# dusk-network/dusk-blindbidproof

Measured on AMD Instinct MI355X. Metric: blind-bid proofs/sec, higher is better.
Workload: dtype u32

## Files before the change

### __graft_entry__.py

```python
import os
import shutil
import subprocess
import sys

ROOT = os.path.dirname(os.path.abspath(__file__))
PKG = os.path.join(ROOT, "dusk_blindbidproof_amd")
CSRC = os.path.join(PKG, "csrc")
LIB = os.path.join(PKG, "libbbp_hip.so")
ORACLE_SO = os.path.join(ROOT, "oracle", "_build", "libbbp_oracle.so")
HOSTCHECK_SO = os.path.join(ROOT, "tests", "_build", "libhostcheck.so")
DEVCHECK_SO = {"chain": os.path.join(ROOT, "tests", "_build", "libbbp_devcheck.so"),
               "nochain": os.path.join(ROOT, "tests", "_build", "libbbp_devcheck_nochain.so")}
DEVCHECK_DEFS = {"chain": [], "nochain": ["-DBBP_FE_NO_CHAIN"]}


def _newer(target, sources):
    if not os.path.exists(target):
        return True
    t = os.path.getmtime(target)
    return any(os.path.getmtime(s) > t for s in sources)


def _run(cmd):
    print("+", " ".join(cmd), flush=True)
    subprocess.check_call(cmd)


def _csrc_files(exts):
    return sorted(os.path.join(CSRC, f) for f in os.listdir(CSRC) if f.endswith(exts))


def build_hip(force=False):
    srcs = _csrc_files((".hip", ".cpp"))
    deps = srcs + _csrc_files((".h", ".inc")) + [os.path.join(ROOT, "include", "bbp.h")]
    if not force and not _newer(LIB, deps):
        return LIB
    hipcc = shutil.which("hipcc") or "/opt/rocm/bin/hipcc"
    objdir = os.path.join(PKG, "build")
    os.makedirs(objdir, exist_ok=True)
    objs = []
    procs = []
    for s in srcs:
        o = os.path.join(objdir, os.path.basename(s) + ".o")
        objs.append(o)
        if force or _newer(o, [s] + _csrc_files((".h", ".inc")) + [os.path.join(ROOT, "include", "bbp.h")]):
            cmd = [hipcc, "--offload-arch=gfx950", "-O3", "-std=c++17", "-fPIC", "-c", s, "-o", o]
            print("+", " ".join(cmd), flush=True)
            procs.append((cmd, subprocess.Popen(cmd)))
    for cmd, p in procs:
        if p.wait() != 0:
            raise subprocess.CalledProcessError(p.returncode, cmd)
    _run([hipcc, "--offload-arch=gfx950", "-shared", "-fPIC", "-o", LIB] + objs)
    return LIB


def stale_artefacts():
    stale = []
    deps = _csrc_files((".hip", ".cpp", ".h", ".inc")) + [os.path.join(ROOT, "include", "bbp.h")]
    if _newer(LIB, deps):
        stale.append(os.path.relpath(LIB, ROOT))
    odir = os.path.join(ROOT, "oracle", "c")
    if _newer(ORACLE_SO, [os.path.join(odir, f) for f in os.listdir(odir)]):
        stale.append(os.path.relpath(ORACLE_SO, ROOT))
    return stale


def build_oracle(force=False):
    src = os.path.join(ROOT, "oracle", "c", "bbp_oracle.c")
    if not os.path.exists(src):
        return None
    deps = [os.path.join(ROOT, "oracle", "c", f) for f in os.listdir(os.path.join(ROOT, "oracle", "c"))]
    if not force and not _newer(ORACLE_SO, deps):
        return ORACLE_SO
    os.makedirs(os.path.dirname(ORACLE_SO), exist_ok=True)
    _run(["gcc", "-O2", "-std=gnu11", "-shared", "-fPIC", "-pthread", "-o", ORACLE_SO, src])
    return ORACLE_SO


def build_hostcheck(force=False):
    src = os.path.join(ROOT, "tests", "host_check.cpp")
    deps = [src] + _csrc_files((".h", ".inc"))
    if not force and not _newer(HOSTCHECK_SO, deps):
        return HOSTCHECK_SO
    os.makedirs(os.path.dirname(HOSTCHECK_SO), exist_ok=True)
    _run(["g++", "-O2", "-std=c++17", "-shared", "-fPIC", "-o", HOSTCHECK_SO, src])
    return HOSTCHECK_SO


ROUNDCHECK_SO = os.path.join(ROOT, "tests", "_build", "libroundcheck.so")


def build_roundcheck(force=False):
    src = os.path.join(ROOT, "tests", "round_bids_check.cpp")
    if force or _newer(ROUNDCHECK_SO, [src] + _csrc_files((".h", ".inc"))):
        os.makedirs(os.path.dirname(ROUNDCHECK_SO), exist_ok=True)
        _run(["g++", "-O2", "-std=c++17", "-shared", "-fPIC", "-o", ROUNDCHECK_SO, src])
    return ROUNDCHECK_SO


def _devcheck_cmd(variant):
    hipcc = shutil.which("hipcc") or "/opt/rocm/bin/hipcc"
    src = os.path.join(ROOT, "tests", "device_check.hip")
    return [hipcc, "--offload-arch=gfx950", "-O3", "-std=c++17", "-fPIC", "-shared"] + DEVCHECK_DEFS[variant] + [src, "-o", DEVCHECK_SO[variant]]


def _devcheck_stale(variant):
    return _newer(DEVCHECK_SO[variant], [os.path.join(ROOT, "tests", "device_check.hip")] + _csrc_files((".h", ".inc")))


def build_devcheck(variant="chain", force=False):
    if force or _devcheck_stale(variant):
        os.makedirs(os.path.dirname(DEVCHECK_SO[variant]), exist_ok=True)
        _run(_devcheck_cmd(variant))
    return DEVCHECK_SO[variant]


def build_devcheck_all(force=False):
    procs = []
    for v in DEVCHECK_SO:
        if force or _devcheck_stale(v):
            os.makedirs(os.path.dirname(DEVCHECK_SO[v]), exist_ok=True)
            cmd = _devcheck_cmd(v)
            print("+", " ".join(cmd), flush=True)
            procs.append((cmd, subprocess.Popen(cmd)))
    for cmd, p in procs:
        if p.wait() != 0:
            raise subprocess.CalledProcessError(p.returncode, cmd)
    return dict(DEVCHECK_SO)


SERVER_BIN = os.path.join(PKG, "server", "bbp-uds-server")
LOADGEN_BIN = os.path.join(PKG, "server", "bbp-uds-loadgen")
STUB_SO = os.path.join(ROOT, "tests", "_build", "libbbp_stub.so")


def build_server(force=False):
    sdir = os.path.join(PKG, "server")
    deps = [os.path.join(sdir, f) for f in os.listdir(sdir) if f.endswith((".cpp", ".h"))] + [os.path.join(ROOT, "include", "bbp.h")]
    for out, src in ((SERVER_BIN, "uds_server.cpp"), (LOADGEN_BIN, "uds_loadgen.cpp")):
        if not os.path.exists(os.path.join(sdir, src)):
            continue
        if force or _newer(out, deps):
            _run(["g++", "-O2", "-std=c++17", "-pthread", "-o", out, os.path.join(sdir, src), "-ldl"])
    return SERVER_BIN


def build_stub_engine(force=False):
    srcs = [os.path.join(ROOT, "tests", "stub_engine.cpp"), os.path.join(CSRC, "submit.cpp")]
    if force or _newer(STUB_SO, srcs + [os.path.join(CSRC, "submit.h"), os.path.join(ROOT, "include", "bbp.h")]):
        os.makedirs(os.path.dirname(STUB_SO), exist_ok=True)
        _run(["g++", "-O2", "-std=c++17", "-shared", "-fPIC", "-pthread", "-o", STUB_SO] + srcs)
    return STUB_SO


SAN_FLAGS = {None: ["-O2"], "asan": ["-O1", "-g", "-fsanitize=address,undefined", "-fno-sanitize-recover=all"], "tsan": ["-O1", "-g", "-fsanitize=thread"]}
SERVER_SAN_BIN = {k: os.path.join(ROOT, "tests", "_build", "bbp-uds-server-" + k) for k in ("asan", "tsan")}
STUB_REFUSING_SO = {k: os.path.join(ROOT, "tests", "_build", "libbbp_stub_refusing%s.so" % ("_" + k if k else "")) for k in (None, "asan", "tsan")}


def build_server_san(kind, force=False):
    sdir = os.path.join(PKG, "server")
    deps = [os.path.join(sdir, f) for f in os.listdir(sdir) if f.endswith((".cpp", ".h"))] + [os.path.join(ROOT, "include", "bbp.h")]
    out = SERVER_SAN_BIN[kind]
    if force or _newer(out, deps):
        os.makedirs(os.path.dirname(out), exist_ok=True)
        _run(["g++"] + SAN_FLAGS[kind] + ["-std=c++17", "-pthread", "-o", out, os.path.join(sdir, "uds_server.cpp"), "-ldl"])
    return out


def build_stub_engine_refusing(kind=None, force=False):
    srcs = [os.path.join(ROOT, "tests", "stub_engine_refusing.cpp"), os.path.join(CSRC, "submit.cpp")]
# ... 34 lines not shown
    src = os.path.join(ROOT, "tests", "batch_layout_san.cpp")
    if force or _newer(BATCH_LAYOUT_SAN_BIN, [src, os.path.join(ROOT, "tests", "host_check.cpp")] + _csrc_files((".h", ".inc"))):
        os.makedirs(os.path.dirname(BATCH_LAYOUT_SAN_BIN), exist_ok=True)
        _run(["g++", "-O1", "-g", "-std=c++17", "-fsanitize=address,undefined", "-fno-sanitize-recover=all", "-o", BATCH_LAYOUT_SAN_BIN, src])
    return BATCH_LAYOUT_SAN_BIN


HEDGE_SAN_BIN = os.path.join(ROOT, "tests", "_build", "hedge_san")


def build_hedge_san(force=False):
    src = os.path.join(ROOT, "tests", "hedge_san.cpp")
    if force or _newer(HEDGE_SAN_BIN, [src] + _csrc_files((".h", ".inc"))):
        os.makedirs(os.path.dirname(HEDGE_SAN_BIN), exist_ok=True)
        _run(["g++", "-O1", "-g", "-std=c++17", "-fsanitize=address,undefined", "-fno-sanitize-recover=all", "-o", HEDGE_SAN_BIN, src])
    return HEDGE_SAN_BIN


STUB_ENTROPY_SO = os.path.join(ROOT, "tests", "_build", "libbbp_stub_entropy.so")


def build_stub_engine_entropy(force=False):
    srcs = [os.path.join(ROOT, "tests", "stub_engine_entropy.cpp"), os.path.join(CSRC, "submit.cpp")]
    if force or _newer(STUB_ENTROPY_SO, srcs + [os.path.join(ROOT, "tests", "stub_engine.cpp"), os.path.join(CSRC, "submit.h"), os.path.join(ROOT, "include", "bbp.h")]):
        os.makedirs(os.path.dirname(STUB_ENTROPY_SO), exist_ok=True)
        _run(["g++", "-O2", "-std=c++17", "-shared", "-fPIC", "-pthread", "-o", STUB_ENTROPY_SO] + srcs)
    return STUB_ENTROPY_SO


COMBINER_TSAN_BIN = os.path.join(ROOT, "tests", "_build", "combiner_tsan")


def build_combiner_tsan(force=False):
    srcs = [os.path.join(ROOT, "tests", "combiner_tsan.cpp"), os.path.join(CSRC, "submit.cpp")]
    if force or _newer(COMBINER_TSAN_BIN, srcs + [os.path.join(CSRC, "submit.h")]):
        os.makedirs(os.path.dirname(COMBINER_TSAN_BIN), exist_ok=True)
        _run(["g++", "-O1", "-g", "-std=c++17", "-fsanitize=thread", "-pthread", "-o", COMBINER_TSAN_BIN] + srcs)
    return COMBINER_TSAN_BIN


COMBINER_RULES_BIN = os.path.join(ROOT, "tests", "_build", "combiner_rules")


def build_combiner_rules(force=False):
    srcs = [os.path.join(ROOT, "tests", "combiner_rules.cpp"), os.path.join(CSRC, "submit.cpp")]
    if force or _newer(COMBINER_RULES_BIN, srcs + [os.path.join(CSRC, "submit.h")]):
        os.makedirs(os.path.dirname(COMBINER_RULES_BIN), exist_ok=True)
        _run(["g++", "-O1", "-std=c++17", "-pthread", "-o", COMBINER_RULES_BIN] + srcs)
    return COMBINER_RULES_BIN


COMBINER_MIXED_BIN = {False: os.path.join(ROOT, "tests", "_build", "combiner_mixed"), True: os.path.join(ROOT, "tests", "_build", "combiner_mixed_tsan")}


def build_combiner_mixed(tsan=False, force=False):
    out = COMBINER_MIXED_BIN[bool(tsan)]
    srcs = [os.path.join(ROOT, "tests", "combiner_mixed.cpp"), os.path.join(CSRC, "submit.cpp")]
    if force or _newer(out, srcs + [os.path.join(CSRC, "submit.h")]):
        os.makedirs(os.path.dirname(out), exist_ok=True)
        flags = ["-O1", "-g", "-fsanitize=thread"] if tsan else ["-O1"]
        _run(["g++"] + flags + ["-std=c++17", "-pthread", "-o", out] + srcs)
    return out


COMBINER_ROUNDS_BIN = {False: os.path.join(ROOT, "tests", "_build", "combiner_rounds"), True: os.path.join(ROOT, "tests", "_build", "combiner_rounds_tsan")}


def build_combiner_rounds(tsan=False, force=False):
    out = COMBINER_ROUNDS_BIN[bool(tsan)]
    srcs = [os.path.join(ROOT, "tests", "combiner_rounds.cpp"), os.path.join(CSRC, "submit.cpp")]
    if force or _newer(out, srcs + [os.path.join(CSRC, "submit.h")]):
        os.makedirs(os.path.dirname(out), exist_ok=True)
        flags = ["-O1", "-g", "-fsanitize=thread"] if tsan else ["-O1"]
        _run(["g++"] + flags + ["-std=c++17", "-pthread", "-o", out] + srcs)
    return out


def build():
    build_hip()
    build_server()
    build_stub_engine()
    build_oracle()
    build_hostcheck()
    build_roundcheck()
    build_devcheck_all()
    sys.path.insert(0, ROOT)
    import dusk_blindbidproof_amd


def smoke():
    sys.path.insert(0, ROOT)
    import dusk_blindbidproof_amd as bbp
    from tests import smoke_case

    smoke_case.run(bbp)


if __name__ == "__main__":
    build()
```

### dusk_blindbidproof_amd/csrc/msm.hip

```cpp
#include "context.h"

namespace bbp {

#ifndef BBP_FOLD_PRIO
#define BBP_FOLD_PRIO 2
#endif
#ifndef BBP_MSM_WAVES
#define BBP_MSM_WAVES 2
#endif
#ifndef BBP_MSM_WAVES_MAX
#define BBP_MSM_WAVES_MAX 2
#endif

#ifdef BBP_MSM_PROF
__device__ unsigned long long g_msm_prof[8];
#define MSM_PROF_BEGIN() unsigned long long prof_t = wall_clock64()
#define MSM_PROF_MARK(i)                                                    \
    if (tid == 0) {                                                         \
        unsigned long long now_ = wall_clock64();                           \
        atomicAdd(&g_msm_prof[i], now_ - prof_t);                           \
        prof_t = now_;                                                      \
    }
#else
#define MSM_PROF_BEGIN()
// ... 94 lines not shown
    __shared__ u32 part[SORT_T];
    const int tid = threadIdx.x;
    if (ticket && blockIdx.x == 0 && tid == 0) *ticket = 0;
    if (n_active && blockIdx.x >= *n_active) return;
    const size_t work = blockIdx.x, msm = work / split;
    const u32 i0 = (u32)(work % split) * n_sub;
    const u32 n = i0 < n_total ? min(n_sub, n_total - i0) : 0u;
    __builtin_amdgcn_s_setprio(3);
    const u32* sbase;
    const u32* base_idx = nullptr;
    u32 base0 = 0;
    if (MODE != 1) {
        const size_t src = msm_map ? (size_t)msm_map[msm] : msm;
        sbase = scal_a + (src * (size_t)n_total + i0) * 8;
        base_idx = aux + (size_t)(msm % n_idx_sets) * n_total + i0;
    } else {
        const u32 side = (u32)msm & 1u;
        sbase = (side ? aux : scal_a) + ((msm >> 1) * (size_t)2048 + i0) * 8;
        base0 = (side ? BBP_BASE_H0 : BBP_BASE_G0) + i0;
    }
    u32* sorted = sorted_all + work * (size_t)n_sub * W;
    auto key = [&](u32 i, u32 mag) -> u32 { return (MODE != 1 ? 0u : ((i0 + i) & (FOLD_CLS - 1)) * FOLD_M) + ((mag + 1) >> 1); };

    for (int k = tid; k <= K; k += SORT_T) cursor[k] = 0;
    __syncthreads();
    for (u32 i = tid; i < n; i += SORT_T) {
        const uint4* sp = reinterpret_cast<const uint4*>(sbase + (size_t)i * 8);
        uint4 lo = sp[0], hi = sp[1];
        const u32 s[8] = {lo.x, lo.y, lo.z, lo.w, hi.x, hi.y, hi.z, hi.w};
        if (MODE != 1 && base_idx[i] == MSM_SKIP_BASE) continue;
        sc_for_each_naf_digit<NAF>(s, [&](u32, u32 mag, u32) { atomicAdd(&cursor[key(i, mag)], 1u); });
    }
    __syncthreads();
    {
        u32 local = 0;
        for (int r = 1; r <= G; r++)
            if (tid * G + r <= K) local += cursor[tid * G + r];
        const int lane = tid & 63, wave = tid >> 6;
        u32 incl = local;
#pragma unroll
        for (int d = 1; d < 64; d <<= 1) {
            const u32 up = (u32)__shfl_up((int)incl, d, 64);
            if (lane >= d) incl += up;
        }
        if (lane == 63) part[wave] = incl;
        __syncthreads();
        if (tid < 64) {
            constexpr int NW = SORT_T / 64;
            u32 v = tid < NW ? part[tid] : 0u, sc_ = v;
#pragma unroll
            for (int d = 1; d < 64; d <<= 1) {
                const u32 up = (u32)__shfl_up((int)sc_, d, 64);
                if (tid >= d) sc_ += up;
            }
            if (tid < NW) part[tid] = sc_ - v;
        }
        __syncthreads();
        u32 base = part[wave] + incl - local;
        for (int r = 1; r <= G; r++) {
            if (tid * G + r > K) break;
            const u32 c = cursor[tid * G + r];
            cursor[tid * G + r] = base;
            base += c;
        }
    }
    __syncthreads();
    for (u32 i = tid; i < n; i += SORT_T) {
        const uint4* sp = reinterpret_cast<const uint4*>(sbase + (size_t)i * 8);
        uint4 lo = sp[0], hi = sp[1];
        const u32 s[8] = {lo.x, lo.y, lo.z, lo.w, hi.x, hi.y, hi.z, hi.w};
        if (MODE != 1 && base_idx[i] == MSM_SKIP_BASE) continue;
        const u32 tb = (MODE != 1 ? base_idx[i] : base0 + i) * MSM_POS;
        sc_for_each_naf_digit<NAF>(s, [&](u32 pos, u32 mag, u32 neg) {
            u32 at = atomicAdd(&cursor[key(i, mag)], 1u);
            sorted[at] = (tb + pos) | (neg << 31);
        });
    }
    __syncthreads();
    u32* cur_out = cursor_all + work * (size_t)(K + 1);
    for (int k = tid; k <= K; k += SORT_T) cur_out[k] = k ? cursor[k] : 0u;
}

template <int MODE> struct sort_cap { static constexpr u32 V = BBP_SORT_CAP; };
template <> struct sort_cap<1> { static constexpr u32 V = 8192; };

template <int MODE>
__global__ __launch_bounds__(SORT_T) void k_msm_sort_staged(const u32* __restrict__ scal_a, const u32* __restrict__ aux, u32 n_total, u32 n_idx_sets,
                                                             u32 n_sub, u32 split, u32* __restrict__ sorted_all, u32* __restrict__ cursor_all,
                                                             const u32* __restrict__ msm_map, const u32* __restrict__ n_active, u32 CAP, u32* __restrict__ ticket) {
    constexpr int K = msm_geom<MODE>::K, NAF = msm_geom<MODE>::NAF, W = msm_geom<MODE>::W, G = K >= SORT_T ? K / SORT_T : 1;
    extern __shared__ u32 stage[];
    __shared__ u32 start[K + 2];
    __shared__ u32 fill[K + 1];
    __shared__ u32 part[SORT_T];
    const int tid = threadIdx.x;
    if (ticket && blockIdx.x == 0 && tid == 0) *ticket = 0;
    if (n_active && blockIdx.x >= *n_active) return;
    const size_t work = blockIdx.x, msm = work / split;
    const u32 i0 = (u32)(work % split) * n_sub;
    const u32 n = i0 < n_total ? min(n_sub, n_total - i0) : 0u;
    __builtin_amdgcn_s_setprio(3);
    const u32* sbase;
    const u32* base_idx = nullptr;
    u32 base0 = 0;
    if (MODE != 1) {
        const size_t src = msm_map ? (size_t)msm_map[msm] : msm;
        sbase = scal_a + (src * (size_t)n_total + i0) * 8;
        base_idx = aux + (size_t)(msm % n_idx_sets) * n_total + i0;
    } else {
        const u32 side = (u32)msm & 1u;
        sbase = (side ? aux : scal_a) + ((msm >> 1) * (size_t)2048 + i0) * 8;
        base0 = (side ? BBP_BASE_H0 : BBP_BASE_G0) + i0;
    }
    u32* sorted = sorted_all + work * (size_t)n_sub * W;
    auto key = [&](u32 i, u32 mag) -> u32 { return (MODE != 1 ? 0u : ((i0 + i) & (FOLD_CLS - 1)) * FOLD_M) + ((mag + 1) >> 1); };

    for (int k = tid; k <= K; k += SORT_T) fill[k] = 0;
    __syncthreads();
    for (u32 i = tid; i < n; i += SORT_T) {
        const uint4* sp = reinterpret_cast<const uint4*>(sbase + (size_t)i * 8);
        uint4 lo = sp[0], hi = sp[1];
        const u32 s[8] = {lo.x, lo.y, lo.z, lo.w, hi.x, hi.y, hi.z, hi.w};
        if (MODE != 1 && base_idx[i] == MSM_SKIP_BASE) continue;
        sc_for_each_naf_digit<NAF>(s, [&](u32, u32 mag, u32) { atomicAdd(&fill[key(i, mag)], 1u); });
    }
    __syncthreads();
    {
        u32 local = 0;
        for (int r = 1; r <= G; r++)
            if (tid * G + r <= K) local += fill[tid * G + r];
        const int lane = tid & 63, wave = tid >> 6;
        u32 incl = local;
#pragma unroll
        for (int d = 1; d < 64; d <<= 1) {
            const u32 up = (u32)__shfl_up((int)incl, d, 64);
            if (lane >= d) incl += up;
        }
        if (lane == 63) part[wave] = incl;
        __syncthreads();
        if (tid < 64) {
            constexpr int NW = SORT_T / 64;
            u32 v = tid < NW ? part[tid] : 0u, sc_ = v;
#pragma unroll
            for (int d = 1; d < 64; d <<= 1) {
                const u32 up = (u32)__shfl_up((int)sc_, d, 64);
                if (tid >= d) sc_ += up;
            }
            if (tid < NW) part[tid] = sc_ - v;
        }
        __syncthreads();
        u32 base = part[wave] + incl - local;
        for (int r = 1; r <= G; r++) {
            if (tid * G + r > K) break;
            const u32 c = fill[tid * G + r];
            start[tid * G + r] = base;
            fill[tid * G + r] = 0;
            base += c;
        }
        if (tid == SORT_T - 1) start[K + 1] = base;
        if (tid == 0) start[0] = 0;
    }
    __syncthreads();
    u32 kb = 1;
    while (kb <= (u32)K) {
        const u32 base = start[kb];
        const bool direct = start[kb + 1] - base > CAP;
        u32 ke = kb + 1;
        if (!direct) {
            u32 lo = kb + 1, hi = (u32)K + 1;
            while (lo < hi) {
                const u32 mid = (lo + hi + 1) >> 1;
                if (start[mid] - base <= CAP) lo = mid; else hi = mid - 1;
            }
            ke = lo;
        }
        if (start[ke] != base) {
            for (u32 i = tid; i < n; i += SORT_T) {
                const uint4* sp = reinterpret_cast<const uint4*>(sbase + (size_t)i * 8);
                uint4 lo4 = sp[0], hi4 = sp[1];
                const u32 s[8] = {lo4.x, lo4.y, lo4.z, lo4.w, hi4.x, hi4.y, hi4.z, hi4.w};
                if (MODE != 1 && base_idx[i] == MSM_SKIP_BASE) continue;
                const u32 tb = (MODE != 1 ? base_idx[i] : base0 + i) * MSM_POS;
                sc_for_each_naf_digit<NAF>(s, [&](u32 pos, u32 mag, u32 neg) {
                    const u32 k = key(i, mag);
                    if (k >= kb && k < ke) {
                        const u32 at = start[k] + atomicAdd(&fill[k], 1u);
                        const u32 ent = (tb + pos) | (neg << 31);
                        if (direct) sorted[at] = ent; else stage[at - base] = ent;
                    }
                });
            }
            __syncthreads();
            if (!direct) {
                const u32 cnt = start[ke] - base;
                for (u32 i = tid; i < cnt; i += SORT_T) sorted[base + i] = stage[i];
            }
            __syncthreads();
        }
        kb = ke;
    }
    u32* cur_out = cursor_all + work * (size_t)(K + 1);
    for (int k = tid; k <= K; k += SORT_T) cur_out[k] = k ? start[k + 1] : 0u;
}

#ifndef BBP_ACC_WG
#define BBP_ACC_WG 256
#endif
constexpr int ACC_WG = BBP_ACC_WG, ACC_WGS = ACC_T / ACC_WG;
static_assert(ACC_T % ACC_WG == 0 && ACC_WG % 64 == 0, "accumulate workgroup geometry");

template <int MODE>
__global__ __launch_bounds__(ACC_WG) __attribute__((amdgpu_waves_per_eu(BBP_MSM_WAVES, BBP_MSM_WAVES_MAX)))
void k_msm_acc(const niels_row* __restrict__ ptable, const u32* __restrict__ sorted_all, const u32* __restrict__ cursor_all, u32 n ,
               ge* __restrict__ bsum_all, ge* __restrict__ psum_all, ge* __restrict__ out, const u32* __restrict__ n_active, u32* __restrict__ fault,
               u32 n_work, u32* __restrict__ ticket) {
    constexpr int K = msm_geom<MODE>::K, W = msm_geom<MODE>::W, G = K / MSM_T;
    __shared__ u32 cursor[K + 1];
#ifdef BBP_ACC_PERSIST
    static_assert(ACC_WGS == 1, "the persistent form draws whole MSMs");
    __shared__ u32 s_ticket;
  for (;;) {
    __syncthreads();
    if (threadIdx.x == 0) s_ticket = atomicAdd(ticket, 1u);
    __syncthreads();
    const size_t msm = s_ticket;
    if (msm >= n_work || (n_active && msm >= *n_active)) return;
    const int tid = (int)threadIdx.x;
#else
    const size_t msm = blockIdx.x / ACC_WGS;
    const int tid = (int)(blockIdx.x % ACC_WGS) * ACC_WG + (int)threadIdx.x;
    if (n_active && msm >= *n_active) return;
#endif
    const u32* sorted = sorted_all + msm * (size_t)n * W;
#ifdef BBP_MSM_PRIO
    __builtin_amdgcn_s_setprio(BBP_MSM_PRIO);
#endif
    MSM_PROF_BEGIN();
    {
        const u32* cur_in = cursor_all + msm * (size_t)(K + 1);
        for (int k = threadIdx.x; k <= K; k += ACC_WG) cursor[k] = cur_in[k];
    }
    __syncthreads();
    MSM_PROF_MARK(1);

    const u32 E = cursor[K];
    ge* bsum = bsum_all + msm * (size_t)K;
    ge* psum = psum_all + msm * (size_t)ACC_T;
#ifdef BBP_KO_ACC_PERMILLE
    const u32 c0 = (u32)(((u64)tid * E) / ACC_T), c1 = c0 + (u32)(((u64)((u32)(((u64)(tid + 1) * E) / ACC_T) - c0) * BBP_KO_ACC_PERMILLE) / 1000);
#else
    const u32 c0 = (u32)(((u64)tid * E) / ACC_T), c1 = (u32)(((u64)(tid + 1) * E) / ACC_T);
#endif
#ifdef BBP_MSM_PROF
    const unsigned long long clk0 = clock64();
#endif
    u32 k_first = 0;
    bool inside = false;
#ifdef BBP_ACC_COOP
    {
        __shared__ __attribute__((aligned(1024))) u8 rowimg[ACC_WG / 64][COOP_IMG];
        const int lane = (int)threadIdx.x & 63;
        u8* wb = rowimg[threadIdx.x >> 6];
        const u32 A = (u32)lane * 128u + ((((u32)lane >> 1) & 7u) << 4);
        const u32 srcoff = (((u32)lane & 7u) ^ (((u32)lane >> 3) >> 1)) << 4;
        const u32 n_it = (E + (u32)ACC_T - 1) / (u32)ACC_T, len = c1 - c0;
        u32 k = 1, kend = 0;
        ge* dest = &psum[tid];
        if (len) {
            u32 lo = 1, hi = K;
            while (lo < hi) {
                u32 mid = (lo + hi) >> 1;
                if (cursor[mid] > c0) hi = mid; else lo = mid + 1;
            }
            k = lo, kend = cursor[k];
            k_first = lo;
            inside = cursor[k - 1] < c0;
            if (!inside) dest = &bsum[k - 1];
        }
        ge acc = ge_identity();
        u32 ent_cur = len ? sorted[c0] : 0u;
        u32 ent_nxt = len > 1 ? sorted[c0 + 1] : 0u;
        if (n_it) coop_issue(ptable, wb, coop_clamp_row(ent_cur, fault), lane, srcoff);
// ... 346 lines not shown
#pragma unroll 1
            for (int i = 0; i < n_dbl; i++) q = ge_dbl(q);
        }
        if (take) v = ge_add(v, q);
    }
    if (l == 0 && valid) out[msm] = v;
}

constexpr int REDUCE_L = 16;
__global__ __launch_bounds__(64) void k_msm_reduce(u32 n_out, u32 split, u32 items, const ge* __restrict__ tmp, ge* __restrict__ out) {
    __builtin_amdgcn_s_setprio(3);
    const u32 t = blockIdx.x * blockDim.x + threadIdx.x;
    const u32 o = t / REDUCE_L, j = t % REDUCE_L;
    const u32 msm = o / items, c = o % items;
    ge acc = ge_identity();
    if (o < n_out && j < split) acc = tmp[((size_t)msm * split + j) * items + c];
    for (u32 jj = j + REDUCE_L; o < n_out && jj < split; jj += REDUCE_L)
        acc = ge_add(acc, tmp[((size_t)msm * split + jj) * items + c]);
#pragma unroll 1
    for (int d = REDUCE_L / 2; d >= 1; d >>= 1) {
        const ge other = ge_shfl_down(acc, d);
        if ((int)j < d) acc = ge_add(acc, other);
    }
    if (o < n_out && j == 0) out[o] = acc;
}


struct MsmScratch {
    u32 *sorted, *cursor;
    ge *bsum, *psum, *tmp;
    u32* ticket;
    size_t bytes;
};
static MsmScratch msm_scratch_layout(void* base, size_t n_msm, size_t n_terms, size_t W, size_t K, size_t out_items = 1) {
    auto up = [](size_t x) { return (x + 255) / 256 * 256; };
    MsmScratch m;
    size_t o = 0;
    m.sorted = reinterpret_cast<u32*>(static_cast<u8*>(base) + o);
    o += up(n_msm * n_terms * W * sizeof(u32));
    m.cursor = reinterpret_cast<u32*>(static_cast<u8*>(base) + o);
    o += up(n_msm * (K + 1) * sizeof(u32));
    m.bsum = reinterpret_cast<ge*>(static_cast<u8*>(base) + o);
    o += n_msm * K * sizeof(ge);
    m.psum = reinterpret_cast<ge*>(static_cast<u8*>(base) + o);
    o += n_msm * ACC_T * sizeof(ge);
    m.tmp = reinterpret_cast<ge*>(static_cast<u8*>(base) + o);
    o += up(n_msm * out_items * sizeof(ge));
    m.ticket = reinterpret_cast<u32*>(static_cast<u8*>(base) + o);
    o += 256;
    m.bytes = o;
    return m;
}
size_t msm_scratch_bytes(uint32_t n_msm, uint32_t n_terms) {
    const u32 split = msm_split(n_msm, n_terms), n_sub = (n_terms + split - 1) / split;
    size_t a = msm_scratch_layout(nullptr, (size_t)n_msm * split, n_sub, MSM_W, MSM_K).bytes;
    if (split > 1) a = std::max(a, msm_scratch_layout(nullptr, (size_t)n_msm * split, n_sub, SMALL_W, SMALL_K).bytes);
    const size_t b = msm_scratch_layout(nullptr, n_msm, n_terms, MSM_W, MSM_K).bytes;
    return a > b ? a : b;
}

static inline u32 acc_grid(bbp_ctx*, u32 n_work) {
#ifdef BBP_ACC_PERSIST
    static const u32 cap = [] { const char* e = getenv("BBP_ACC_PERSIST_GRID"); return e ? (u32)atoi(e) : 512u; }();
    return n_work < cap ? n_work : cap;
#else
    return n_work * ACC_WGS;
#endif
}

int32_t fold_generators_launch(bbp_ctx* ctx, uint32_t n_proofs, const sc* g_dev, const sc* h_dev, ge* out_dev, hipStream_t stream,
                               int scratch_slot) {
    if (n_proofs == 0) return BBP_OK;
    const size_t n_msm = 2 * (size_t)n_proofs;
    const u32 split = msm_split((u32)n_msm, 2048), n_sub = (2048 + split - 1) / split;
    const size_t n_work = n_msm * split;
    DevBuf& scratch = ctx->slice_fold[scratch_slot];
    int32_t rc = dev_reserve(ctx, scratch, msm_scratch_layout(nullptr, n_work, n_sub, FOLD_W, FOLD_K, FOLD_CLS).bytes);
    if (rc) return rc;
    const MsmScratch m = msm_scratch_layout(scratch.p, n_work, n_sub, FOLD_W, FOLD_K, FOLD_CLS);
    {
        ScopedEvent ev(ctx, TAG_MSM_SORT, stream);
        if (ctx->msm_knobs.sort_staged & 2) {
            if (!ctx->sort_lds_attr1) {
                BBP_HIP_TRY(ctx, hipFuncSetAttribute((const void*)k_msm_sort_staged<1>, hipFuncAttributeMaxDynamicSharedMemorySize, (int)(sort_cap<1>::V * 4)));
                ctx->sort_lds_attr1 = true;
            }
            hipLaunchKernelGGL(k_msm_sort_staged<1>, dim3((u32)n_work), dim3(SORT_T), sort_cap<1>::V * 4, stream, (const u32*)g_dev, (const u32*)h_dev, 2048u, 1u,
                               n_sub, split, m.sorted, m.cursor, (const u32*)nullptr, (const u32*)nullptr, sort_cap<1>::V, m.ticket);
        } else
            hipLaunchKernelGGL(k_msm_sort<1>, dim3((u32)n_work), dim3(SORT_T), 0, stream, (const u32*)g_dev, (const u32*)h_dev, 2048u, 1u, n_sub, split,
                               m.sorted, m.cursor, (const u32*)nullptr, (const u32*)nullptr, m.ticket);
        BBP_HIP_TRY(ctx, hipGetLastError());
    }
    {
        ScopedEvent ev(ctx, TAG_MSM, stream);
        hipLaunchKernelGGL(k_msm_acc<1>, dim3(acc_grid(ctx, (u32)n_work)), dim3(ACC_WG), 0, stream, ctx->ptable, m.sorted, m.cursor, n_sub, m.bsum, m.psum,
                           split > 1 ? m.tmp : out_dev, (const u32*)nullptr, ctx->health, (u32)n_work, m.ticket);
        BBP_HIP_TRY(ctx, hipGetLastError());
    }
    ScopedEvent evf(ctx, TAG_MSM_FOLD, stream);
    hipLaunchKernelGGL(k_msm_fold<1>, dim3((u32)n_work), dim3(MSM_T), 0, stream, m.cursor, m.bsum, m.psum, split > 1 ? m.tmp : out_dev,
                       (const u32*)nullptr);
    BBP_HIP_TRY(ctx, hipGetLastError());
    if (split > 1) {
        const u32 n_out = (u32)n_msm * FOLD_CLS;
        hipLaunchKernelGGL(k_msm_reduce, dim3((n_out * REDUCE_L + 63) / 64), dim3(64), lds_token(ctx), stream, n_out, split, (u32)FOLD_CLS, m.tmp, out_dev);
        BBP_HIP_TRY(ctx, hipGetLastError());
    }
    return BBP_OK;
}

__global__ __launch_bounds__(64) void k_encode(const ge* __restrict__ pts, u32 n, u32* __restrict__ out_words) {
    u32 i = blockIdx.x * blockDim.x + threadIdx.x;
    if (i >= n) return;
    ge p = pts[i];
    u32 w[8];
    ge_encode_words(w, p);
    uint4* o = reinterpret_cast<uint4*>(out_words + (size_t)i * 8);
    o[0] = make_uint4(w[0], w[1], w[2], w[3]);
    o[1] = make_uint4(w[4], w[5], w[6], w[7]);
}

__global__ void k_debug_poke(u32* sorted) { sorted[0] = 0x7ffffff0u; }

int32_t msm_launch(bbp_ctx* ctx, uint32_t n_msm, uint32_t n_terms, const u32* scalars_dev, const u32* base_idx_dev,
                   ge* out_points_dev, hipStream_t stream, uint32_t n_idx_sets, int scratch_slot, const u32* msm_map_dev,
                   const u32* n_active_dev, bool chain_acc) {
    if (n_msm == 0) return BBP_OK;
    if (n_terms == 0 || n_terms > 65535u) {
        ctx->err = "msm_launch: n_terms out of range";
        return BBP_ERR_BAD_ARG;
    }
    DevBuf& scratch = scratch_slot ? ctx->slice_sorted[scratch_slot] : ctx->sorted;
    int32_t rc = dev_reserve(ctx, scratch, msm_scratch_bytes(n_msm, n_terms));
    if (rc) return rc;
    const MsmPlan plan = plan_msm(ctx->msm_knobs, n_msm, n_terms, n_active_dev != nullptr);
    const u32 split = plan.split, n_sub = plan.n_sub, n_work = plan.n_work;
    if (plan.geom == MsmPlan::SMALL) {
        const MsmScratch ms = msm_scratch_layout(scratch.p, n_work, n_sub, SMALL_W, SMALL_K);
        {
            ScopedEvent ev(ctx, TAG_MSM_SORT, stream);
            hipLaunchKernelGGL(k_msm_sort<2>, dim3(n_work), dim3(SORT_T), 0, stream, scalars_dev, base_idx_dev, n_terms, n_idx_sets, n_sub, split, ms.sorted, ms.cursor,
                               msm_map_dev, n_active_dev, ms.ticket);
            BBP_HIP_TRY(ctx, hipGetLastError());
        }
        if (ctx->debug_corrupt) {
            ctx->debug_corrupt = 0;
            hipLaunchKernelGGL(k_debug_poke, dim3(1), dim3(1), 0, stream, ms.sorted);
            BBP_HIP_TRY(ctx, hipGetLastError());
        }
        {
            ScopedEvent ev(ctx, TAG_MSM, stream);
            hipLaunchKernelGGL(k_msm_acc<2>, dim3(acc_grid(ctx, n_work)), dim3(ACC_WG), 0, stream, ctx->ptable, ms.sorted, ms.cursor, n_sub, ms.bsum, ms.psum, ms.tmp,
                               n_active_dev, ctx->health, n_work, ms.ticket);
            BBP_HIP_TRY(ctx, hipGetLastError());
        }
        {
            ScopedEvent evf(ctx, TAG_MSM_FOLD, stream);
            hipLaunchKernelGGL(k_msm_fold<2>, dim3(n_work), dim3(MSM_T), 0, stream, ms.cursor, ms.bsum, ms.psum, ms.tmp, n_active_dev);
            BBP_HIP_TRY(ctx, hipGetLastError());
        }
        hipLaunchKernelGGL(k_msm_reduce, dim3((n_msm * REDUCE_L + 63) / 64), dim3(64), lds_token(ctx), stream, n_msm, split, 1u, ms.tmp, out_points_dev);
        BBP_HIP_TRY(ctx, hipGetLastError());
        return BBP_OK;
    }
    const MsmScratch m = msm_scratch_layout(scratch.p, n_work, n_sub, MSM_W, MSM_K);
    {
        ScopedEvent ev(ctx, TAG_MSM_SORT, stream);
        if (plan.sort != MsmPlan::PLAIN) {
            const u32 cap = plan.sort_cap;
            if (!ctx->sort_lds_attr) {
                BBP_HIP_TRY(ctx, hipFuncSetAttribute((const void*)k_msm_sort_staged<0>, hipFuncAttributeMaxDynamicSharedMemorySize, (int)(SORT_CAP_WIDE * 4)));
                ctx->sort_lds_attr = true;
            }
            hipLaunchKernelGGL(k_msm_sort_staged<0>, dim3(n_work), dim3(SORT_T), cap * 4, stream, scalars_dev, base_idx_dev, n_terms, n_idx_sets, n_sub, split,
                               m.sorted, m.cursor, msm_map_dev, n_active_dev, cap, m.ticket);
        }
        else
            hipLaunchKernelGGL(k_msm_sort<0>, dim3(n_work), dim3(SORT_T), 0, stream, scalars_dev, base_idx_dev, n_terms, n_idx_sets, n_sub, split,
                               m.sorted, m.cursor, msm_map_dev, n_active_dev, m.ticket);
        BBP_HIP_TRY(ctx, hipGetLastError());
    }
    if (ctx->debug_corrupt) {
        ctx->debug_corrupt = 0;
        hipLaunchKernelGGL(k_debug_poke, dim3(1), dim3(1), 0, stream, m.sorted);
        BBP_HIP_TRY(ctx, hipGetLastError());
    }
    chain_acc = chain_acc && ctx->verify_serial_acc;
    if (chain_acc && ctx->vacc_valid)
        BBP_HIP_TRY(ctx, hipStreamWaitEvent(stream, ctx->ev_vacc[ctx->vacc_seq % bbp_ctx::VACC_RING], 0));
    {
        ScopedEvent ev(ctx, TAG_MSM, stream);
        hipLaunchKernelGGL(k_msm_acc<0>, dim3(acc_grid(ctx, n_work)), dim3(ACC_WG), 0, stream, ctx->ptable, m.sorted, m.cursor, n_sub, m.bsum, m.psum,
                           split > 1 ? m.tmp : out_points_dev, n_active_dev, ctx->health, n_work, m.ticket);
        BBP_HIP_TRY(ctx, hipGetLastError());
    }
    static const bool chain_after_fold = getenv("BBP_VERIFY_CHAIN_AFTER_FOLD") && atoi(getenv("BBP_VERIFY_CHAIN_AFTER_FOLD"));
    if (chain_acc && !chain_after_fold) {
        ctx->vacc_seq++;
        BBP_HIP_TRY(ctx, hipEventRecord(ctx->ev_vacc[ctx->vacc_seq % bbp_ctx::VACC_RING], stream));
        ctx->vacc_valid = true;
    }
    ScopedEvent evf(ctx, TAG_MSM_FOLD, stream);
    if (plan.fold == MsmPlan::HALF)
        hipLaunchKernelGGL(k_msm_fold_half, dim3((n_work + 1) / 2), dim3(64), 0, stream, m.cursor, m.bsum, m.psum, split > 1 ? m.tmp : out_points_dev,
                           n_work, n_active_dev);
    else
        hipLaunchKernelGGL(k_msm_fold<0>, dim3(n_work), dim3(MSM_T), 0, stream, m.cursor, m.bsum, m.psum, split > 1 ? m.tmp : out_points_dev, n_active_dev);
    BBP_HIP_TRY(ctx, hipGetLastError());
    if (chain_acc && chain_after_fold) {
        ctx->vacc_seq++;
        BBP_HIP_TRY(ctx, hipEventRecord(ctx->ev_vacc[ctx->vacc_seq % bbp_ctx::VACC_RING], stream));
        ctx->vacc_valid = true;
    }
    if (plan.reduce) {
        hipLaunchKernelGGL(k_msm_reduce, dim3((n_msm * REDUCE_L + 63) / 64), dim3(64), lds_token(ctx), stream, n_msm, split, 1u, m.tmp, out_points_dev);
        BBP_HIP_TRY(ctx, hipGetLastError());
    }
#ifdef BBP_MSM_PROF
    static int launches = 0;
    if (++launches % 16 == 0) {
        unsigned long long h[8];
        (void)hipStreamSynchronize(stream);
        (void)hipMemcpyFromSymbol(h, HIP_SYMBOL(g_msm_prof), sizeof h);
        fprintf(stderr, "[msm prof, %d launches, 10ns ticks of lane 0 summed over WGs] load %llu D1 %llu D1wait %llu D2 %llu E %llu; D1 shader clock %.0f MHz\n", launches,
                h[1], h[2], h[3], h[4], h[5], 100.0 * (double)h[6] / (double)h[2]);
    }
#endif
    return BBP_OK;
}

int32_t encode_launch(bbp_ctx* ctx, uint32_t n, const ge* pts_dev, uint8_t* out32_dev, hipStream_t stream) {
    if (n == 0) return BBP_OK;
    ScopedEvent ev(ctx, TAG_ENCODE, stream);
    hipLaunchKernelGGL(k_encode, dim3((n + 63) / 64), dim3(64), lds_token(ctx), stream, pts_dev, n, (u32*)out32_dev);
    BBP_HIP_TRY(ctx, hipGetLastError());
    return BBP_OK;
}

}
```

### dusk_blindbidproof_amd/csrc/msm_plan.h

```cpp
#pragma once
#include <stdint.h>
#include <stdlib.h>
#include <string.h>

#include <initializer_list>

namespace bbp {

constexpr int MSM_NAF = 12;
constexpr int MSM_W = 22;
constexpr int MSM_K = 1 << (MSM_NAF - 2);
constexpr int SMALL_NAF = 9;
constexpr int SMALL_K = 1 << (SMALL_NAF - 2);
constexpr int SMALL_W = 29;

#ifndef BBP_SORT_CAP
#define BBP_SORT_CAP 21504
#endif
constexpr uint32_t SORT_CAP_WIDE = 32768;
constexpr uint32_t SORT_WIDE_FROM = 3000;
constexpr uint32_t MSM_SPLIT_MAX = 16;

struct MsmKnobs {
    int sort_staged = 3;
    int fold_half_from = 512;
    int msm_small = 1;
    uint32_t split_below = 128;
    uint32_t split_target = 512;

    bool set(const char* name, const char* text) {
        const int v = atoi(text);
        if (!strcmp(name, "BBP_SORT_STAGED")) sort_staged = v & 7;
        else if (!strcmp(name, "BBP_FOLD_HALF_FROM")) fold_half_from = v < 1 ? 1 : v;
        else if (!strcmp(name, "BBP_MSM_SMALL")) msm_small = v != 0;
        else if (!strcmp(name, "BBP_MSM_SPLIT_BELOW")) split_below = (uint32_t)v;
        else if (!strcmp(name, "BBP_MSM_SPLIT_TARGET")) split_target = (uint32_t)v;
        else return false;
        return true;
    }
    static const MsmKnobs& process() {
        static const MsmKnobs once = [] {
            MsmKnobs k;
            for (const char* name : {"BBP_MSM_SPLIT_BELOW", "BBP_MSM_SPLIT_TARGET"})
                if (const char* text = getenv(name)) k.set(name, text);
            return k;
        }();
        return once;
    }
    static MsmKnobs from_env() {
        MsmKnobs k = process();
        for (const char* name : {"BBP_SORT_STAGED", "BBP_FOLD_HALF_FROM", "BBP_MSM_SMALL"})
            if (const char* text = getenv(name)) k.set(name, text);
        return k;
    }
};

inline uint32_t msm_split(const MsmKnobs& k, uint32_t n_msm, uint32_t n_terms) {
    if (n_msm >= k.split_below) return 1;
    uint32_t s = k.split_target / n_msm;
    if (s > MSM_SPLIT_MAX) s = MSM_SPLIT_MAX;
    while (s > 1 && n_terms / s < 128) s--;
    return s ? s : 1;
}
inline uint32_t msm_split(uint32_t n_msm, uint32_t n_terms) { return msm_split(MsmKnobs::process(), n_msm, n_terms); }

struct MsmPlan {
    enum Geom { LARGE, SMALL };
    enum Sort { PLAIN, STAGED, STAGED_WIDE };
    enum Fold { LANES128, HALF, SMALL_FOLD };
    uint32_t split = 1;
    uint32_t n_sub = 0;
    uint32_t n_work = 0;
    Geom geom = LARGE;
    Sort sort = PLAIN;
    uint32_t sort_cap = 0;
    Fold fold = LANES128;
    bool reduce = false;

    uint32_t K() const { return geom == SMALL ? SMALL_K : MSM_K; }
    uint32_t W() const { return geom == SMALL ? SMALL_W : MSM_W; }
    uint32_t naf() const { return geom == SMALL ? SMALL_NAF : MSM_NAF; }
};

inline MsmPlan plan_msm(const MsmKnobs& k, uint32_t n_msm, uint32_t n_terms, bool device_sized) {
    MsmPlan p;
    p.split = device_sized ? 1u : msm_split(k, n_msm, n_terms);
    p.n_sub = (n_terms + p.split - 1) / p.split;
    p.n_work = n_msm * p.split;
    p.reduce = p.split > 1;
    if (p.split > 1 && k.msm_small) {
        p.geom = MsmPlan::SMALL;
        p.fold = MsmPlan::SMALL_FOLD;
        return p;
    }
    const bool wide = p.n_sub > SORT_WIDE_FROM;
    if ((k.sort_staged & 1) && (!wide || (k.sort_staged & 4))) {
        p.sort = wide ? MsmPlan::STAGED_WIDE : MsmPlan::STAGED;
        p.sort_cap = wide ? SORT_CAP_WIDE : (uint32_t)BBP_SORT_CAP;
    }
    p.fold = p.n_work >= (uint32_t)k.fold_half_from ? MsmPlan::HALF : MsmPlan::LANES128;
    return p;
}

}
```

### dusk_blindbidproof_amd/csrc/scalar.h

```cpp
#pragma once
#include "field.h"

namespace bbp {

struct sc {
    u32 v[8];
};

#define BBP_SC_LIT(a0, a1, a2, a3, a4, a5, a6, a7) \
    sc { { a0, a1, a2, a3, a4, a5, a6, a7 } }

BBP_HD sc sc_zero() { return BBP_SC_LIT(0, 0, 0, 0, 0, 0, 0, 0); }
BBP_HD sc sc_one() { return BBP_SC_LIT(1, 0, 0, 0, 0, 0, 0, 0); }
BBP_HD sc sc_l() { return BBP_SC_LIT(0x5cf5d3edu, 0x5812631au, 0xa2f79cd6u, 0x14def9deu, 0, 0, 0, 0x10000000u); }
BBP_HD sc sc_rr() { return BBP_SC_LIT(0x449c0f01u, 0xa40611e3u, 0x68859347u, 0xd00e1ba7u, 0x17f5be65u, 0xceec73d2u, 0x7c309a3du, 0x0399411bu); }
BBP_HD sc sc_r() { return BBP_SC_LIT(0x8d98951du, 0xd6ec3174u, 0x737dcf70u, 0xc6ef5bf4u, 0xfffffffeu, 0xffffffffu, 0xffffffffu, 0x0fffffffu); }
#define BBP_SC_LFACTOR 0x12547e1bu

BBP_HD sc sc_from_u32(u32 x) { return BBP_SC_LIT(x, 0, 0, 0, 0, 0, 0, 0); }
BBP_HD sc sc_from_u64(u64 x) { return BBP_SC_LIT((u32)x, (u32)(x >> 32), 0, 0, 0, 0, 0, 0); }

BBP_HD sc sc_cond_sub_l(const sc& a, u32 hi) {
    sc l = sc_l(), t;
    int64_t c = 0;
// ... 217 lines not shown
            i64 cf = tu * f.v[0] + tv * g.v[0], cg = tq * f.v[0] + tr * g.v[0];
            cf >>= 30;
            cg >>= 30;
#pragma unroll
            for (int i = 1; i < 9; i++) {
                const i64 fi = f.v[i], gi = g.v[i];
                cf += tu * fi + tv * gi;
                cg += tq * fi + tr * gi;
                f.v[i - 1] = (i32)cf & M30;
                cf >>= 30;
                g.v[i - 1] = (i32)cg & M30;
                cg >>= 30;
            }
            f.v[8] = (i32)cf;
            g.v[8] = (i32)cg;
        }
    }
    {
        i32 cond_add = d.v[8] >> 31;
#pragma unroll
        for (int i = 0; i < 9; i++) d.v[i] += MOD[i] & cond_add;
        const i32 cond_neg = f.v[8] >> 31;
#pragma unroll
        for (int i = 0; i < 9; i++) d.v[i] = (d.v[i] ^ cond_neg) - cond_neg;
#pragma unroll
        for (int i = 0; i < 8; i++) {
            d.v[i + 1] += d.v[i] >> 30;
            d.v[i] &= M30;
        }
        cond_add = d.v[8] >> 31;
#pragma unroll
        for (int i = 0; i < 9; i++) d.v[i] += MOD[i] & cond_add;
#pragma unroll
        for (int i = 0; i < 8; i++) {
            d.v[i + 1] += d.v[i] >> 30;
            d.v[i] &= M30;
        }
    }
    sc out;
#pragma unroll
    for (int w = 0; w < 8; w++) {
        const int o = 32 * w, li = o / 30, sh = o % 30;
        u64 two = (u64)(u32)d.v[li] | (li + 1 < 9 ? (u64)(u32)d.v[li + 1] << 30 : 0ull);
        if (li + 2 < 9) two |= (u64)(u32)d.v[li + 2] << 60;
        out.v[w] = (u32)(two >> sh);
    }
    return out;
}

BBP_HD void sc_tobytes(uint8_t* out, const sc& a) {
#pragma unroll
    for (int i = 0; i < 8; i++) {
        out[4 * i + 0] = (uint8_t)(a.v[i]);
        out[4 * i + 1] = (uint8_t)(a.v[i] >> 8);
        out[4 * i + 2] = (uint8_t)(a.v[i] >> 16);
        out[4 * i + 3] = (uint8_t)(a.v[i] >> 24);
    }
}

template <int WID, class F>
BBP_HD void sc_for_each_naf_digit(const u32 (&s)[8], F&& f) {
    u32 carry = 0;
    int off = 0;
#pragma unroll
    for (int wi = 0; wi < 8; wi++) {
        const u64 win = (u64)s[wi] | (wi + 1 < 8 ? (u64)s[wi + 1] << 32 : 0ull);
        while (off < 32) {
            const u64 rest = (win ^ (carry ? ~0ull : 0ull)) >> off;
            if (rest == 0) {
                off = 64;
                break;
            }
            off += __builtin_ctzll(rest);
            if (off >= 32) break;
            const u32 t = ((u32)(win >> off) & ((1u << WID) - 1u)) + carry;
            carry = t >> (WID - 1);
            f((u32)(32 * wi + off), carry ? (1u << WID) - t : t, carry);
            off += WID;
        }
        off -= 32;
    }
}

}
```

Measured before the change: 22770.

## Keep packed NAF digits in registers across staged sort passes and batch bucket windows

The staged MSM sort kernel now decodes each scalar's NAF digits once into packed 16-bit slots held in registers, using S items per thread chosen by template. Later scatter passes replay those registers instead of reloading scalars from global memory and re-running the digit decoder for every bucket window. Bucket windows are also planned up front by one wave, up to 62 per round, so the per-window binary search is not redone by every thread. In exchange the kernel uses more registers, n_sub is capped at 5120 for the staged path (larger inputs fall back to the plain sort), and optional profiling counters are added.

```diff
diff --git a/__graft_entry__.py b/__graft_entry__.py
--- a/__graft_entry__.py
+++ b/__graft_entry__.py
@@ -87,6 +87,17 @@
     return HOSTCHECK_SO
 
 
+SORTCHECK_SO = os.path.join(ROOT, "tests", "_build", "libsortcheck.so")
+
+
+def build_sortcheck(force=False):
+    src = os.path.join(ROOT, "tests", "sort_digits_check.cpp")
+    if force or _newer(SORTCHECK_SO, [src] + _csrc_files((".h", ".inc"))):
+        os.makedirs(os.path.dirname(SORTCHECK_SO), exist_ok=True)
+        _run(["g++", "-O2", "-std=c++17", "-shared", "-fPIC", "-o", SORTCHECK_SO, src])
+    return SORTCHECK_SO
+
+
 ROUNDCHECK_SO = os.path.join(ROOT, "tests", "_build", "libroundcheck.so")
 
 
@@ -287,6 +298,7 @@
     build_stub_engine()
     build_oracle()
     build_hostcheck()
+    build_sortcheck()
     build_roundcheck()
     build_devcheck_all()
     sys.path.insert(0, ROOT)
diff --git a/dusk_blindbidproof_amd/csrc/msm.hip b/dusk_blindbidproof_amd/csrc/msm.hip
--- a/dusk_blindbidproof_amd/csrc/msm.hip
+++ b/dusk_blindbidproof_amd/csrc/msm.hip
@@ -200,13 +200,32 @@
 }
 
 template <int MODE> struct sort_cap { static constexpr u32 V = BBP_SORT_CAP; };
-template <> struct sort_cap<1> { static constexpr u32 V = 8192; };
-
-template <int MODE>
+#ifndef BBP_SORT_CAP_FOLD
+#define BBP_SORT_CAP_FOLD 8192
+#endif
+template <> struct sort_cap<1> { static constexpr u32 V = BBP_SORT_CAP_FOLD; };
+constexpr int SORT_S = 3, SORT_S_WIDE = 5, SORT_S_FOLD = 2;
+constexpr int SORT_MAXW = 62;
+static_assert((u32)SORT_S_WIDE * SORT_T >= SORT_STAGED_MAX_TERMS && SORT_S_FOLD * SORT_T >= 2048 && SORT_MAXW + 2 <= SORT_T, "staged sort geometry");
+
+#ifdef BBP_MSM_PROF
+__device__ unsigned long long g_sort_prof[4][16];
+#define SORT_PROF_MARK(i)                                                   \
+    if (tid == 0) {                                                         \
+        unsigned long long now_ = wall_clock64();                           \
+        atomicAdd(&g_sort_prof[prof_cls][(i) < 15 ? (i) : 14], now_ - prof_t); \
+        prof_t = now_;                                                      \
+    }
+#else
+#define SORT_PROF_MARK(i)
+#endif
+
+template <int MODE, int S>
 __global__ __launch_bounds__(SORT_T) void k_msm_sort_staged(const u32* __restrict__ scal_a, const u32* __restrict__ aux, u32 n_total, u32 n_idx_sets,
                                                              u32 n_sub, u32 split, u32* __restrict__ sorted_all, u32* __restrict__ cursor_all,
                                                              const u32* __restrict__ msm_map, const u32* __restrict__ n_active, u32 CAP, u32* __restrict__ ticket) {
     constexpr int K = msm_geom<MODE>::K, NAF = msm_geom<MODE>::NAF, W = msm_geom<MODE>::W, G = K >= SORT_T ? K / SORT_T : 1;
+    constexpr int P = naf_slots<NAF>::P, NSLOT = naf_slots<NAF>::N, DW = naf_slots<NAF>::WORDS;
     extern __shared__ u32 stage[];
     __shared__ u32 start[K + 2];
     __shared__ u32 fill[K + 1];
@@ -233,16 +252,35 @@
     u32* sorted = sorted_all + work * (size_t)n_sub * W;
     auto key = [&](u32 i, u32 mag) -> u32 { return (MODE != 1 ? 0u : ((i0 + i) & (FOLD_CLS - 1)) * FOLD_M) + ((mag + 1) >> 1); };
 
+#ifdef BBP_MSM_PROF
+    const int prof_cls = MODE == 1 ? 3 : n_sub <= 2049 ? 0 : n_sub <= SORT_WIDE_FROM ? 1 : 2;
+    if (tid == 0) atomicAdd(&g_sort_prof[prof_cls][15], 1ull);
+    unsigned long long prof_t = wall_clock64();
+#endif
     for (int k = tid; k <= K; k += SORT_T) fill[k] = 0;
     __syncthreads();
-    for (u32 i = tid; i < n; i += SORT_T) {
-        const uint4* sp = reinterpret_cast<const uint4*>(sbase + (size_t)i * 8);
-        uint4 lo = sp[0], hi = sp[1];
-        const u32 s[8] = {lo.x, lo.y, lo.z, lo.w, hi.x, hi.y, hi.z, hi.w};
-        if (MODE != 1 && base_idx[i] == MSM_SKIP_BASE) continue;
-        sc_for_each_naf_digit<NAF>(s, [&](u32, u32 mag, u32) { atomicAdd(&fill[key(i, mag)], 1u); });
-    }
-    __syncthreads();
+    u32 dig[S][DW], valid[S], tb[S], koff[S];
+#pragma unroll
+    for (int j = 0; j < S; j++) {
+        const u32 i = (u32)tid + (u32)j * SORT_T;
+        valid[j] = 0, tb[j] = 0, koff[j] = 0;
+#pragma unroll
+        for (int d = 0; d < DW; d++) dig[j][d] = 0;
+        if (i < n) {
+            const uint4* sp = reinterpret_cast<const uint4*>(sbase + (size_t)i * 8);
+            uint4 lo = sp[0], hi = sp[1];
+            const u32 s[8] = {lo.x, lo.y, lo.z, lo.w, hi.x, hi.y, hi.z, hi.w};
+            const u32 b = MODE != 1 ? base_idx[i] : base0 + i;
+            if (MODE == 1 || b != MSM_SKIP_BASE) {
+                tb[j] = b * MSM_POS;
+                koff[j] = key(i, 0);
+                const u32 ko = koff[j];
+                sc_naf_digits_packed<NAF>(s, dig[j], valid[j], [&](u32 p) { atomicAdd(&fill[ko + naf_packed_bucket(p)], 1u); });
+            }
+        }
+    }
+    __syncthreads();
+    SORT_PROF_MARK(0);
     {
         u32 local = 0;
         for (int r = 1; r <= G; r++)
@@ -279,43 +317,65 @@
         if (tid == 0) start[0] = 0;
     }
     __syncthreads();
-    u32 kb = 1;
-    while (kb <= (u32)K) {
-        const u32 base = start[kb];
-        const bool direct = start[kb + 1] - base > CAP;
-        u32 ke = kb + 1;
-        if (!direct) {
-            u32 lo = kb + 1, hi = (u32)K + 1;
-            while (lo < hi) {
-                const u32 mid = (lo + hi + 1) >> 1;
-                if (start[mid] - base <= CAP) lo = mid; else hi = mid - 1;
-            }
-            ke = lo;
-        }
-        if (start[ke] != base) {
-            for (u32 i = tid; i < n; i += SORT_T) {
-                const uint4* sp = reinterpret_cast<const uint4*>(sbase + (size_t)i * 8);
-                uint4 lo4 = sp[0], hi4 = sp[1];
-                const u32 s[8] = {lo4.x, lo4.y, lo4.z, lo4.w, hi4.x, hi4.y, hi4.z, hi4.w};
-                if (MODE != 1 && base_idx[i] == MSM_SKIP_BASE) continue;
-                const u32 tb = (MODE != 1 ? base_idx[i] : base0 + i) * MSM_POS;
-                sc_for_each_naf_digit<NAF>(s, [&](u32 pos, u32 mag, u32 neg) {
-                    const u32 k = key(i, mag);
-                    if (k >= kb && k < ke) {
+    u32 kb0 = 1;
+    while (kb0 <= (u32)K) {
+        if (tid < 64) {
+            u32 kb = kb0, nw = 0;
+            while (kb <= (u32)K && nw < (u32)SORT_MAXW) {
+                const u32 base = start[kb];
+                u32 ke = kb + 1;
+                if (start[ke] - base <= CAP) {
+                    u32 lo = kb + 1, hi = (u32)K + 1;
+                    while (lo < hi) {
+                        const u32 mid = (lo + hi + 1) >> 1;
+                        if (start[mid] - base <= CAP) lo = mid; else hi = mid - 1;
+                    }
+                    ke = lo;
+                }
+                if (start[ke] != base) {
+                    if (tid == 0) part[1 + nw] = ke;
+                    nw++;
+                }
+                kb = ke;
+            }
+            if (tid == 0) part[0] = nw, part[1 + nw] = kb;
+        }
+        __syncthreads();
+        SORT_PROF_MARK(2);
+        const u32 nw = (u32)__builtin_amdgcn_readfirstlane((int)part[0]);
+        u32 kb = kb0;
+        for (u32 w = 0; w < nw; w++) {
+            const u32 ke = (u32)__builtin_amdgcn_readfirstlane((int)part[1 + w]);
+            const u32 base = (u32)__builtin_amdgcn_readfirstlane((int)start[kb]), cnt = (u32)__builtin_amdgcn_readfirstlane((int)start[ke]) - base;
+            const bool direct = cnt > CAP;
+#pragma unroll
+            for (int j = 0; j < S; j++) {
+                asm volatile("" : "+v"(valid[j]));
+#pragma unroll
+                for (int d = 0; d < DW; d++) asm volatile("" : "+v"(dig[j][d]));
+                if (!valid[j]) continue;
+#pragma unroll
+                for (int t = 0; t < NSLOT; t++) {
+                    if (!(valid[j] >> t & 1)) continue;
+                    const u32 p = naf_slot<NAF>(dig[j], t), k = koff[j] + naf_packed_bucket(p);
+                    if (k - kb < ke - kb) {
                         const u32 at = start[k] + atomicAdd(&fill[k], 1u);
-                        const u32 ent = (tb + pos) | (neg << 31);
+                        const u32 ent = (tb[j] + naf_packed_pos(p, t / P)) | (naf_packed_neg(p) << 31);
                         if (direct) sorted[at] = ent; else stage[at - base] = ent;
                     }
-                });
+                }
             }
             __syncthreads();
+            SORT_PROF_MARK(3 + 2 * w);
             if (!direct) {
-                const u32 cnt = start[ke] - base;
                 for (u32 i = tid; i < cnt; i += SORT_T) sorted[base + i] = stage[i];
-            }
-            __syncthreads();
-        }
-        kb = ke;
+                __syncthreads();
+            }
+            SORT_PROF_MARK(4 + 2 * w);
+            kb = ke;
+        }
+        kb0 = (u32)__builtin_amdgcn_readfirstlane((int)part[1 + nw]);
+        __syncthreads();
     }
     u32* cur_out = cursor_all + work * (size_t)(K + 1);
     for (int k = tid; k <= K; k += SORT_T) cur_out[k] = k ? start[k + 1] : 0u;
@@ -828,10 +888,10 @@
         ScopedEvent ev(ctx, TAG_MSM_SORT, stream);
         if (ctx->msm_knobs.sort_staged & 2) {
             if (!ctx->sort_lds_attr1) {
-                BBP_HIP_TRY(ctx, hipFuncSetAttribute((const void*)k_msm_sort_staged<1>, hipFuncAttributeMaxDynamicSharedMemorySize, (int)(sort_cap<1>::V * 4)));
+                BBP_HIP_TRY(ctx, hipFuncSetAttribute((const void*)k_msm_sort_staged<1, SORT_S_FOLD>, hipFuncAttributeMaxDynamicSharedMemorySize, (int)(sort_cap<1>::V * 4)));
                 ctx->sort_lds_attr1 = true;
             }
-            hipLaunchKernelGGL(k_msm_sort_staged<1>, dim3((u32)n_work), dim3(SORT_T), sort_cap<1>::V * 4, stream, (const u32*)g_dev, (const u32*)h_dev, 2048u, 1u,
+            hipLaunchKernelGGL((k_msm_sort_staged<1, SORT_S_FOLD>), dim3((u32)n_work), dim3(SORT_T), sort_cap<1>::V * 4, stream, (const u32*)g_dev, (const u32*)h_dev, 2048u, 1u,
                                n_sub, split, m.sorted, m.cursor, (const u32*)nullptr, (const u32*)nullptr, sort_cap<1>::V, m.ticket);
         } else
             hipLaunchKernelGGL(k_msm_sort<1>, dim3((u32)n_work), dim3(SORT_T), 0, stream, (const u32*)g_dev, (const u32*)h_dev, 2048u, 1u, n_sub, split,
@@ -916,11 +976,20 @@
         if (plan.sort != MsmPlan::PLAIN) {
             const u32 cap = plan.sort_cap;
             if (!ctx->sort_lds_attr) {
-                BBP_HIP_TRY(ctx, hipFuncSetAttribute((const void*)k_msm_sort_staged<0>, hipFuncAttributeMaxDynamicSharedMemorySize, (int)(SORT_CAP_WIDE * 4)));
+                BBP_HIP_TRY(ctx, hipFuncSetAttribute((const void*)k_msm_sort_staged<0, SORT_S>, hipFuncAttributeMaxDynamicSharedMemorySize, (int)(SORT_CAP_WIDE * 4)));
+                BBP_HIP_TRY(ctx, hipFuncSetAttribute((const void*)k_msm_sort_staged<0, SORT_S_WIDE>, hipFuncAttributeMaxDynamicSharedMemorySize, (int)(SORT_CAP_WIDE * 4)));
                 ctx->sort_lds_attr = true;
             }
-            hipLaunchKernelGGL(k_msm_sort_staged<0>, dim3(n_work), dim3(SORT_T), cap * 4, stream, scalars_dev, base_idx_dev, n_terms, n_idx_sets, n_sub, split,
-                               m.sorted, m.cursor, msm_map_dev, n_active_dev, cap, m.ticket);
+            if (n_sub > (u32)SORT_S_WIDE * SORT_T) {
+                ctx->err = "msm_launch: staged sort planned for more terms than its lanes hold";
+                return BBP_ERR_INTERNAL;
+            }
+            if (n_sub <= (u32)SORT_S * SORT_T)
+                hipLaunchKernelGGL((k_msm_sort_staged<0, SORT_S>), dim3(n_work), dim3(SORT_T), cap * 4, stream, scalars_dev, base_idx_dev, n_terms, n_idx_sets, n_sub, split,
+                                   m.sorted, m.cursor, msm_map_dev, n_active_dev, cap, m.ticket);
+            else
+                hipLaunchKernelGGL((k_msm_sort_staged<0, SORT_S_WIDE>), dim3(n_work), dim3(SORT_T), cap * 4, stream, scalars_dev, base_idx_dev, n_terms, n_idx_sets, n_sub, split,
+                                   m.sorted, m.cursor, msm_map_dev, n_active_dev, cap, m.ticket);
         }
         else
             hipLaunchKernelGGL(k_msm_sort<0>, dim3(n_work), dim3(SORT_T), 0, stream, scalars_dev, base_idx_dev, n_terms, n_idx_sets, n_sub, split,
@@ -966,8 +1035,15 @@
 #ifdef BBP_MSM_PROF
     static int launches = 0;
     if (++launches % 16 == 0) {
-        unsigned long long h[8];
+        unsigned long long h[8], sp[4][16];
         (void)hipStreamSynchronize(stream);
+        (void)hipMemcpyFromSymbol(sp, HIP_SYMBOL(g_sort_prof), sizeof sp);
+        for (int c = 0; c < 4; c++) {
+            if (!sp[c][15]) continue;
+            fprintf(stderr, "[sort prof class %d, %llu workgroups, 10ns ticks of lane 0 per workgroup]", c, sp[c][15]);
+            for (int i = 0; i < 15; i++) fprintf(stderr, " %.1f", (double)sp[c][i] / (double)sp[c][15]);
+            fprintf(stderr, "\n");
+        }
         (void)hipMemcpyFromSymbol(h, HIP_SYMBOL(g_msm_prof), sizeof h);
         fprintf(stderr, "[msm prof, %d launches, 10ns ticks of lane 0 summed over WGs] load %llu D1 %llu D1wait %llu D2 %llu E %llu; D1 shader clock %.0f MHz\n", launches,
                 h[1], h[2], h[3], h[4], h[5], 100.0 * (double)h[6] / (double)h[2]);
diff --git a/dusk_blindbidproof_amd/csrc/msm_plan.h b/dusk_blindbidproof_amd/csrc/msm_plan.h
--- a/dusk_blindbidproof_amd/csrc/msm_plan.h
+++ b/dusk_blindbidproof_amd/csrc/msm_plan.h
@@ -19,6 +19,7 @@
 #endif
 constexpr uint32_t SORT_CAP_WIDE = 32768;
 constexpr uint32_t SORT_WIDE_FROM = 3000;
+constexpr uint32_t SORT_STAGED_MAX_TERMS = 5120;
 constexpr uint32_t MSM_SPLIT_MAX = 16;
 
 struct MsmKnobs {
@@ -94,7 +95,7 @@
         return p;
     }
     const bool wide = p.n_sub > SORT_WIDE_FROM;
-    if ((k.sort_staged & 1) && (!wide || (k.sort_staged & 4))) {
+    if ((k.sort_staged & 1) && (!wide || (k.sort_staged & 4)) && p.n_sub <= SORT_STAGED_MAX_TERMS) {
         p.sort = wide ? MsmPlan::STAGED_WIDE : MsmPlan::STAGED;
         p.sort_cap = wide ? SORT_CAP_WIDE : (uint32_t)BBP_SORT_CAP;
     }
diff --git a/dusk_blindbidproof_amd/csrc/scalar.h b/dusk_blindbidproof_amd/csrc/scalar.h
--- a/dusk_blindbidproof_amd/csrc/scalar.h
+++ b/dusk_blindbidproof_amd/csrc/scalar.h
@@ -323,4 +323,49 @@
     }
 }
 
-}
+template <int WID> struct naf_slots {
+    static_assert(WID >= 8 && WID <= 12, "a slot is 16 bits and `valid` has 32");
+    static constexpr int P = (32 + WID - 1) / WID, N = 8 * P, WORDS = N / 2;
+};
+BBP_HD constexpr u32 naf_pack(u32 pos, u32 mag, u32 neg) { return (pos & 31u) | ((mag >> 1) << 5) | (neg << 15); }
+BBP_HD constexpr u32 naf_packed_pos(u32 p, u32 word) { return 32u * word + (p & 31u); }
+BBP_HD constexpr u32 naf_packed_bucket(u32 p) { return ((p >> 5) & 0x3ffu) + 1u; }
+BBP_HD constexpr u32 naf_packed_neg(u32 p) { return (p >> 15) & 1u; }
+template <int WID> BBP_HD constexpr u32 naf_slot(const u32 (&dig)[naf_slots<WID>::WORDS], int slot) { return (dig[slot >> 1] >> (16 * (slot & 1))) & 0xffffu; }
+
+template <int WID, class F>
+BBP_HD void sc_naf_digits_packed(const u32 (&s)[8], u32 (&dig)[naf_slots<WID>::WORDS], u32& valid, F&& each) {
+    constexpr int P = naf_slots<WID>::P;
+#pragma unroll
+    for (int d = 0; d < naf_slots<WID>::WORDS; d++) dig[d] = 0;
+    valid = 0;
+    u32 carry = 0;
+    int off = 0;
+#pragma unroll
+    for (int wi = 0; wi < 8; wi++) {
+        const u64 win = (u64)s[wi] | (wi + 1 < 8 ? (u64)s[wi + 1] << 32 : 0ull);
+#pragma unroll
+        for (int t = 0; t < P; t++) {
+            if (off < 32) {
+                const u64 rest = (win ^ (carry ? ~0ull : 0ull)) >> off;
+                if (rest == 0) {
+                    off = 64;
+                } else {
+                    off += __builtin_ctzll(rest);
+                    if (off < 32) {
+                        const u32 v = ((u32)(win >> off) & ((1u << WID) - 1u)) + carry;
+                        carry = v >> (WID - 1);
+                        const u32 p = naf_pack((u32)off, carry ? (1u << WID) - v : v, carry);
+                        dig[(wi * P + t) >> 1] |= p << (16 * ((wi * P + t) & 1));
+                        each(p);
+                        valid |= 1u << (wi * P + t);
+                        off += WID;
+                    }
+                }
+            }
+        }
+        off -= 32;
+    }
+}
+
+}
```

Result: faster. 23450 (median of 6 runs) (+3.0%).
